# LeSN-Lab/diff-ViT

Measured on AMD Instinct MI355X. Metric: images/sec DeiT-S int8 224^2 b=256 (quantized forward), higher is better.
Workload: dtype int8; 1 GPU; deit_small PoT-PTQ forward, bit_config=[8]*50, 224x224, batch 256 per GPU; global_batch=256, parallelism=dp1, streams_per_gpu=3, collective=none, ranks_seen=1, distinct_devices=1

## Files before the change

diff-vit_amd/csrc/p2vit_attn.hip:

```cpp
#include "p2vit_attn_lis.h"

#define WA_HD 32
#define WA_KEYS 64
#define WA_DEAD(kb, r) (NT > 0 && (kb) * 16 + (r) >= NT)
#define WA_PAD(kb, r) (!(NT > 0 && (kb) * 16 + 12 + (r) < NT))
template <int NT, bool TAP>
__global__ __launch_bounds__(256, 3) void k_window_attention(std::conditional_t<TAP, WinAttnArgs, WinAttnKArgs> a) {
  constexpr int VSTRIDE = WA_KEYS + 4;
  __shared__ __attribute__((aligned(16))) int8_t sK[4][WA_KEYS * WA_HD];
  __shared__ __attribute__((aligned(16))) unsigned short sVt[4][WA_HD * VSTRIDE];
  __shared__ float sT[4][232];
  __shared__ __attribute__((aligned(16))) unsigned short sP[4][4][16];
  __shared__ unsigned short sMeta[WA_KEYS + 16];
  __shared__ long long lutE[258];
  __shared__ double lutFR[258];
  const int tid = threadIdx.x, lane = tid & 63, wave = tid >> 6, g = lane >> 4, l15 = lane & 15;
  const int ws = a.wa.ws, N = ws * ws, nW = a.wa.n_windows;
  const int hgroups = (a.H + 3) >> 2;
  const int blk = blockIdx.x;
  const int hg = blk % hgroups, w = (blk / hgroups) % nW, b = blk / (hgroups * nW);
  const int head = hg * 4 + wave;
  const int C = a.H * WA_HD;
  const long long ldq = a.wa.qkv_stride ? a.wa.qkv_stride : 3 * C, ldo = a.wa.out_stride ? a.wa.out_stride : C;
  const bool hok = head < a.H;
// ... 220 lines not shown
              const int k = (int)((__float_as_uint(ratio[e]) + 0x00400000u) >> 23) - 127;
              const long long trow = (((long long)b * nW + w) * a.H + head) * N + qi;
              if (a.probs_k) a.probs_k[trow * N + kb * 16 + 4 * g + r] = (int8_t)(k > 16 ? 16 : k);
              if (a.probs_kp) a.probs_kp[trow * a.pitch + kb * 16 + 4 * g + r] = (int8_t)(k > 16 ? 16 : k);
            }
          }
          pk[e2] = lis_prob_pair(ratio[0], ratio[1]);
        }
        pb[p] = (v4i){(int)pk[0], (int)pk[1], (int)pk[2], (int)pk[3]};
      }
    }
    v4f o[2] = {(v4f){0.f, 0.f, 0.f, 0.f}, (v4f){0.f, 0.f, 0.f, 0.f}};
#pragma unroll
    for (int p = 0; p < 2; ++p) {
      const v8bf fb = __builtin_bit_cast(v8bf, pb[p]);
#pragma unroll
      for (int dt = 0; dt < 2; ++dt) {
        const unsigned short* vp = &sVt[wave][(dt * 16 + l15) * VSTRIDE + p * 32 + 4 * g];
        const uint2 lo = *reinterpret_cast<const uint2*>(vp);
        const uint2 hi = *reinterpret_cast<const uint2*>(vp + 16);
        v4i va = {(int)lo.x, (int)lo.y, (int)hi.x, (int)hi.y};
        o[dt] = __builtin_amdgcn_mfma_f32_16x16x32_bf16(__builtin_bit_cast(v8bf, va), fb, o[dt], 0, 0, 0);
      }
    }
    if (qi < N) {
      int8_t* dst = a.out + ((long long)b * a.T + rowq) * ldo + head * WA_HD + 4 * g;
#pragma unroll
      for (int dt = 0; dt < 2; ++dt)
        *reinterpret_cast<unsigned*>(dst + dt * 16) = pack4_rne_sat(o[dt][0] * av_mul, o[dt][1] * av_mul, o[dt][2] * av_mul, o[dt][3] * av_mul);
    }
  }
}


int g_attn_waves = 8;
int p2v_launch_window_attention_wide(const WinAttnArgs& a, hipStream_t st);
template <int NT, bool TAP>
static void launch_window_t(const WinAttnArgs& a, dim3 grid, hipStream_t st) {
  hipLaunchKernelGGL((k_window_attention<NT, TAP>), grid, dim3(256), 0, st, a);
}
int p2v_launch_window_attention(const WinAttnArgs& a, hipStream_t st) {
  if (a.wa.ws > 8) return p2v_launch_window_attention_wide(a, st);
  const int hgroups = (a.H + 3) / 4;
  const dim3 grid((unsigned)(a.B * a.wa.n_windows * hgroups));
  static void (*const table[2][2])(const WinAttnArgs&, dim3, hipStream_t) = {{launch_window_t<49, true>, launch_window_t<49, false>},
                                                                             {launch_window_t<0, true>, launch_window_t<0, false>}};
  table[a.wa.ws == 7 ? 0 : 1][a.tapped() ? 0 : 1](a, grid, st);
  CHECK_LAUNCH();
  return 0;
}

int p2v_launch_attention_wide(const AttnArgs& a, int head_dim, int nkb, hipStream_t st);

int g_attn_stream = 0;
int g_attn_packed = 1;
int p2v_attention_kernel_of(int head_dim, int tokens, int tapped) {
  const int resident = p2v_resident_tokens_of(head_dim);
  if (!resident || tokens <= 0 || tokens > P2V_MAX_TOKENS_STREAMED) return -1;
  if (g_attn_stream) return P2V_KERNEL_STREAMING;
  if (tokens <= resident) return P2V_KERNEL_RESIDENT;
  if (g_attn_packed && head_dim == 64 && !tapped && tokens <= P2V_MAX_TOKENS_PACKED) return P2V_KERNEL_PACKED;
  return P2V_KERNEL_STREAMING;
}

int p2v_launch_attention(const AttnArgs& a, int head_dim, hipStream_t st) {
  const int nkb = (a.N + 31) / 32;
  {
    int ex;
    const float m2 = a.at.s_qkv_sq * a.at.inv_s_attn;
    if (!(m2 > 0.f) || frexpf(m2, &ex) != 0.5f) return -2;
  }
  switch (p2v_attention_kernel_of(head_dim, a.N, a.tapped())) {
    case P2V_KERNEL_RESIDENT: break;
    case P2V_KERNEL_PACKED: return p2v_launch_attention_packed(a, st);
    case P2V_KERNEL_STREAMING: return p2v_launch_attention_stream(a, head_dim, st);
    default: return -1;
  }
  if (head_dim == 64) return launch_attn_hd<64, 19, true>(a, nkb, st);
  if (head_dim == 32) return launch_attn_hd<32, 19, false>(a, nkb, st);
  return p2v_launch_attention_wide(a, head_dim, nkb, st);
}
```

diff-vit_amd/csrc/p2vit_attn_lis.h:

```cpp
#pragma once
#include "p2vit_device.h"
#include "p2vit_launch.h"

extern int g_attn_waves;


#define P2V_PROB_SCALE 0x1p111f
__device__ __forceinline__ unsigned lis_prob_pair(float r0, float r1) {
  const unsigned hi2 = __builtin_amdgcn_perm(__float_as_uint(r1), __float_as_uint(r0), 0x07060302u);
  const unsigned eb = __builtin_bit_cast(unsigned, __builtin_bit_cast(v2u16, hi2) + (v2u16){0x40, 0x40}) & 0x7F807F80u;
  unsigned out;
  asm("v_pk_sub_u16 %0, %1, %2 clamp" : "=v"(out) : "s"(0x47804780u), "v"(eb));
  return out;
}

__device__ __forceinline__ void lis_table_entry(const p2v_attn& at, int t, long long* lutE, double* lutFR) {
  if (t >= 256) {
    lutE[256] = 0;
    lutFR[256] = 1.0;
    return;
  }
  int xi = -t;
  const int lim = 32 * at.x0_int;
  xi = xi < lim ? lim : xi;
  const int q = xi / at.x0_int;
  const int r = xi - at.x0_int * q;
  const long long z = (long long)r * (r + at.b_int) + at.c_int;
  long long e = z << (32 - q);
  e = e < 0 ? 0 : e;
  lutE[t] = e;
  lutFR[t] = 1.0 / (double)(float)e;
}

#ifdef P2V_DIAG
extern unsigned long long* g_gemm_stamps;
#define AT_STAMP(slot)                                                                                             \
  do {                                                                                                             \
    if (a.stamps && threadIdx.x == 0 && (slot) < 16) a.stamps[(long long)blockIdx.x * 16 + (slot)] = __builtin_readcyclecounter(); \
  } while (0)
#else
#define AT_STAMP(slot) do { } while (0)
#endif
template <int HD, int NKP, bool TAP, bool ISH>
__global__ __launch_bounds__(512, HD > 64 ? 2 : (NKP <= 7 ? 4 : (NKP <= 10 ? 3 : 2))) void k_lis_attention(std::conditional_t<TAP, AttnArgs, AttnKArgs> a) {
  static_assert(HD % 16 == 0 && HD >= 16 && HD <= 128, "head_dim");
  constexpr int KROWS = NKP * 32;
  constexpr int NKB = NKP * 2;
  constexpr int VSTRIDE = KROWS + 4;
  constexpr int CH = HD / 16;
  constexpr int NQ = (CH + 3) / 4;
  constexpr int NDT = HD / 16;
  extern __shared__ __attribute__((aligned(16))) unsigned char smem[];
  int8_t* sK = reinterpret_cast<int8_t*>(smem);
  unsigned short* sVt = reinterpret_cast<unsigned short*>(smem + KROWS * HD);
  unsigned char* lutE = smem + KROWS * HD + HD * VSTRIDE * 2;
  unsigned char* lutFR = lutE + 258 * 8;
  typedef __attribute__((address_space(3))) const long long* lds_i64p;
  typedef __attribute__((address_space(3))) const double* lds_f64p;
  const int ebase = (int)(unsigned)(uintptr_t)(__attribute__((address_space(3))) unsigned char*)lutE;

  const int tid = threadIdx.x, lane = tid & 63, wave = tid >> 6, g = lane >> 4, l15 = lane & 15;
  const int b = blockIdx.x / a.H, head = blockIdx.x % a.H;
  const int N = a.N, D = a.H * HD, ld = 3 * D;
  const int8_t* base = a.qkv + (long long)b * N * ld + head * HD;
  AT_STAMP(0);

  if (tid < 256) {
    int xi = -tid;
    const int lim = 32 * a.at.x0_int;
    xi = xi < lim ? lim : xi;
    const int q = xi / a.at.x0_int;
    const int r = xi - a.at.x0_int * q;
    const long long z = (long long)r * (r + a.at.b_int) + a.at.c_int;
    long long e = z << (32 - q);
    e = e < 0 ? 0 : e;
    const float ef = (float)e;
    reinterpret_cast<long long*>(lutE)[tid] = e;
    reinterpret_cast<double*>(lutFR)[tid] = 1.0 / (double)ef;
    if (tid == 0) {
      reinterpret_cast<long long*>(lutE)[256] = 0;
      reinterpret_cast<double*>(lutFR)[256] = 1.0;
    }
  }
  AT_STAMP(1);
  for (int i0 = tid; i0 < KROWS * CH; i0 += 2 * (int)blockDim.x) {
    uint4 kv[2], vv[2];
#pragma unroll
    for (int u = 0; u < 2; ++u) {
      const int i = i0 + u * (int)blockDim.x;
      const int row = i / CH, c = i % CH;
      kv[u] = make_uint4(0, 0, 0, 0);
      vv[u] = make_uint4(0, 0, 0, 0);
      if (i < KROWS * CH && row < N) {
        kv[u] = *reinterpret_cast<const uint4*>(base + (long long)row * ld + D + c * 16);
        vv[u] = *reinterpret_cast<const uint4*>(base + (long long)row * ld + 2 * D + c * 16);
      }
    }
#pragma unroll
    for (int u = 0; u < 2; ++u) {
      const int i = i0 + u * (int)blockDim.x;
      if (i >= KROWS * CH) break;
      const int row = i / CH, c = i % CH;
      const int sw = (HD == 64) ? (c ^ (((row >> 3) & 1) << 1)) : c;
      *reinterpret_cast<uint4*>(sK + row * HD + sw * 16) = kv[u];
      const unsigned w4[4] = {vv[u].x, vv[u].y, vv[u].z, vv[u].w};
#pragma unroll
      for (int j = 0; j < 16; ++j) {
        const float f = (float)sx8(w4[j >> 2], j & 3);
        sVt[(c * 16 + j) * VSTRIDE + row] = (unsigned short)(__float_as_uint(f) >> 16);
      }
    }
  }

  const float nmm = -(a.at.qk_scale * (a.at.s_qkv_sq * a.at.inv_s_attn));
  const float avm = a.at.av_mul * P2V_PROB_SCALE;
  const int nqb = ((a.nq > 0 && a.nq < N ? a.nq : N) + 15) >> 4;
  const int nwaves = (int)(blockDim.x >> 6);
  AT_STAMP(2);
  v4i fq_next[NQ];
#pragma unroll
  for (int j = 0; j < NQ; ++j) {
    fq_next[j] = (v4i){0, 0, 0, 0};
    if (4 * j + g < CH && wave < nqb) {
      const int qr0 = wave * 16 + l15;
      fq_next[j] = *reinterpret_cast<const v4i*>(base + (long long)(qr0 < N ? qr0 : N - 1) * ld + (4 * j + g) * 16);
    }
  }
  __syncthreads();
  AT_STAMP(3);
  [[maybe_unused]] int stamp_base = 4;
  for (int qb = wave; qb < nqb; qb += nwaves) {
    const int qrow = qb * 16 + l15;
    v4i fq[NQ];
#pragma unroll
    for (int j = 0; j < NQ; ++j) {
      fq[j] = fq_next[j];
      if (4 * j + g < CH && qb + nwaves < nqb) {
        const int qn = (qb + nwaves) * 16 + l15;
        fq_next[j] = *reinterpret_cast<const v4i*>(base + (long long)(qn < N ? qn : N - 1) * ld + (4 * j + g) * 16);
      }
    }
    v4i s[NKB];
#pragma unroll
    for (int kb = 0; kb < NKB; ++kb) {
      const int row = kb * 16 + l15;
#pragma unroll
      for (int j = 0; j < NQ; ++j) {
        const bool live = 4 * j + g < CH;
        const int c = live ? 4 * j + g : 0;
        const int sw = (HD == 64) ? (c ^ (((row >> 3) & 1) << 1)) : c;
        v4i fk = *reinterpret_cast<const v4i*>(sK + row * HD + sw * 16);
        if (!live) fk = (v4i){0, 0, 0, 0};
        if (j == 0) s[kb] = __builtin_amdgcn_mfma_i32_16x16x64_i8(fk, fq[0], (v4i){0, 0, 0, 0}, 0, 0, 0);
        else s[kb] = __builtin_amdgcn_mfma_i32_16x16x64_i8(fk, fq[j], s[kb], 0, 0, 0);
      }
    }
    const bool tail_empty = (NKB - 1) * 16 >= N;
#ifdef P2V_DIAG
    asm volatile("s_nop 0" :: "v"(s[NKB - 1][0]));
#endif
    AT_STAMP(stamp_base);
    long long S = 0;
    [[maybe_unused]] int rowmax = 0;
    if (ISH) {
      const int p = a.pshift, hm1 = (1 << (p - 1)) - 1;
      int mx = -100000;
#pragma unroll
      for (int kb = 0; kb < NKB; ++kb) {
        if (kb == NKB - 1 && tail_empty) continue;
#pragma unroll
        for (int r = 0; r < 4; ++r) {
          const int sv = s[kb][r];
          int code = (int)((unsigned)sv + (unsigned)hm1 + (((unsigned)sv >> p) & 1u)) >> p;
          code = code < -128 ? -128 : (code > 127 ? 127 : code);
          if (kb >= NKB - 2) code = (kb * 16 + 4 * g + r) < N ? code : -100000;
          s[kb][r] = code;
          mx = code > mx ? code : mx;
        }
      }
      {
        int o = __shfl_xor(mx, 16);
        mx = o > mx ? o : mx;
        o = __shfl_xor(mx, 32);
        mx = o > mx ? o : mx;
      }
      if (TAP) rowmax = mx;
      const int mx8 = (mx << 3) + ebase;
#pragma unroll
      for (int kb = 0; kb < NKB; ++kb) {
        if (kb == NKB - 1 && tail_empty) continue;
#pragma unroll
        for (int r = 0; r < 4; ++r) {
          int d8;
          asm("v_mad_i32_i24 %0, %1, -8, %2" : "=v"(d8) : "v"(s[kb][r]), "v"(mx8));
          if (kb >= NKB - 2) d8 = d8 > ebase + 2048 ? ebase + 2048 : d8;
          s[kb][r] = d8;
          S += *(lds_i64p)(uintptr_t)(unsigned)d8;
        }
        __builtin_amdgcn_sched_barrier(0);
      }
    } else {
    int mn = 1000;
#pragma unroll
    for (int kb = 0; kb < NKB; ++kb) {
      if (kb == NKB - 1 && tail_empty) continue;
#pragma unroll
      for (int r = 0; r < 4; ++r) {
        int nc = (int)__builtin_amdgcn_fmed3f(rintf((float)s[kb][r] * nmm), -127.f, 128.f);
        if (kb >= NKB - 2) nc = (kb * 16 + 4 * g + r) < N ? nc : 1000;
        s[kb][r] = nc;
        mn = nc < mn ? nc : mn;
      }
    }
    {
      int o = __shfl_xor(mn, 16);
      mn = o < mn ? o : mn;
      o = __shfl_xor(mn, 32);
      mn = o < mn ? o : mn;
    }
    if (TAP) rowmax = -mn;
    const int neg8mn = -8 * mn + ebase;
#pragma unroll
    for (int kb = 0; kb < NKB; ++kb) {
      if (kb == NKB - 1 && tail_empty) continue;
#pragma unroll
      for (int r = 0; r < 4; ++r) {
        int d8 = (s[kb][r] << 3) + neg8mn;
        if (kb >= NKB - 2) d8 = d8 > ebase + 2048 ? ebase + 2048 : d8;
        s[kb][r] = d8;
        S += *(lds_i64p)(uintptr_t)(unsigned)d8;
      }
      __builtin_amdgcn_sched_barrier(0);
    }
    }
    S += __shfl_xor(S, 16);
    S += __shfl_xor(S, 32);
    const float Sf = (float)S;
    const double Sd = (double)Sf;
    AT_STAMP(stamp_base + 1);

// ... 99 lines not shown
```

diff-vit_amd/csrc/p2vit_capi.cpp:

```cpp
#include <hip/hip_runtime.h>
#include <math.h>
#include <stdarg.h>
#include <stdio.h>
#include <stdlib.h>
#include <string.h>

#include <initializer_list>
#include <memory>
#include <vector>

#include "p2vit_kernels.h"

static thread_local char g_err[512] = "";

static int fail(int code, const char* fmt, ...) {
  va_list ap;
  va_start(ap, fmt);
  vsnprintf(g_err, sizeof g_err, fmt, ap);
  va_end(ap);
  return code;
}
struct KeepLastError {
  char keep[sizeof g_err];
  KeepLastError() { memcpy(keep, g_err, sizeof keep); }
// ... 7 lines not shown
}
static inline int round_up(int v, int m) { return (v + m - 1) / m * m; }
static bool is_pot(float v) {
  int ex;
  return v > 0.f && frexpf(v, &ex) == 0.5f;
}

static int check_lis_consts(const char* who, int x0_int, int b_int, int c_int) {
  if (x0_int >= 0) return fail(P2V_E_ARG, "%s: x0_int must be negative", who);
  if (c_int <= 0 || c_int >= (1 << 24) || b_int < 0 || b_int >= (1 << 23) || x0_int < -(1 << 12))
    return fail(P2V_E_UNSUPPORTED, "%s: log-int-softmax constants out of range (x0 %d, b %d, c %d): softmax input scale below 2^-11?", who, x0_int,
                b_int, c_int);
  return P2V_OK;
}
static int check_requant_scale(const char* who, float inv_s_out) {
  if (!(is_pot(inv_s_out) && inv_s_out >= 0x1p-40f && inv_s_out <= 0x1p40f))
    return fail(P2V_E_UNSUPPORTED, "%s: REQUANT 1/scale %g must be a power of two (it is folded into the column scales)", who, inv_s_out);
  return P2V_OK;
}
static int check_gelu_tab(const char* who, const p2v_gelu_tab& t) {
  if (t.table && (t.cells <= 0 || t.cells > 4096)) return fail(P2V_E_ARG, "%s: GELU table with %d cells", who, t.cells);
  return P2V_OK;
}
static int check_attn(const char* who, const p2v_attn& at) {
  const int rc = check_lis_consts(who, at.x0_int, at.b_int, at.c_int);
  if (rc != P2V_OK) return rc;
  if (!is_pot(at.s_qkv_sq * at.inv_s_attn)) return fail(P2V_E_UNSUPPORTED, "%s: s_qkv_sq * inv_s_attn must be a power of two", who);
  if (!(at.qk_scale > 0.f) || !(at.av_mul > 0.f)) return fail(P2V_E_ARG, "%s: qk_scale and av_mul must be positive", who);
  if (!is_pot(at.av_mul) || at.av_mul > 0x1p15f || at.av_mul < 0x1p-40f)
    return fail(P2V_E_UNSUPPORTED, "%s: av_mul %g must be a power of two in [2^-40, 2^15]", who, at.av_mul);
  return P2V_OK;
}

struct p2v_plan {
  p2v_model_desc d;
  int tokens, patches, k_patch, k_patch_pad, n_layers;
  std::vector<p2v_linear> lin[2];
  std::vector<char> lin_set[2];
  float inv_s_input;
  p2v_epilogue embed_epi;
  const int8_t* cls_codes;
  const int8_t* embed_cls_codes = nullptr;
  bool embed_set;
  std::vector<p2v_block> blocks;
  std::vector<char> block_set;
  p2v_ln final_ln;
  float head_inv_s, head_s;
  bool head_set;
  std::vector<float*> ln_pre_buf;
  float* final_pre_buf = nullptr;
  std::vector<char> block_folded;
  std::vector<const float*> resid_tab;
  std::vector<float*> resid_buf;
  int device = -1;
  ~p2v_plan() {
    int prev = -1;
    const bool sw = device >= 0 && hipGetDevice(&prev) == hipSuccess && prev != device && hipSetDevice(device) == hipSuccess;
    for (float* b : ln_pre_buf)
      if (b) (void)hipFree(b);
    for (float* b : resid_buf)
      if (b) (void)hipFree(b);
    if (final_pre_buf) (void)hipFree(final_pre_buf);
    if (sw) (void)hipSetDevice(prev);
  }
};

static void build_resid_tables(p2v_plan* plan, int block);
static int bit_index(int bits) { return bits == 4 ? 0 : (bits == 8 ? 1 : -1); }
template <class Block>
static auto& block_ln(Block& b, int i) { return i < 2 ? b.ln1[i] : b.ln2[(i - 2) >> 1][(i - 2) & 1]; }
static bool ln_constants_present(const p2v_ln& l, bool with_mask = true) {
  return (l.mask || !with_mask) && l.gamma && l.beta && l.inv_out && l.post_mul;
}

extern "C" {

extern int g_ln_generic;
extern int g_ln_rows;
extern int g_attn_waves;
extern int g_ln_gemm;
extern int g_ln_gemm_ver;
extern int g_gemm_tile;
extern int g_resid_pre;
extern int g_attn_stream;
extern int g_attn_packed;
extern int g_ln_pre;
extern int g_gemm_rows;
int g_cls_rows = 1;

enum { ANY_ENV = 1, ANY_API = 2 };
static const struct Switch {
  const char *name, *env;
  int* var;
  int lo, hi, step, any;
  bool takes(int v, int how) const { return (any & how) || (v >= lo && v <= hi && (v - lo) % step == 0); }
  void set(int v) const { *var = (hi == 1 && lo == 0) ? v != 0 : v; }
} kSwitches[] = {
    {"attn_waves", "P2V_ATTN_WAVES", &g_attn_waves, 4, 8, 1, 0},
    {"ln_gemm", "P2V_LN_GEMM", &g_ln_gemm, 0, 1, 1, ANY_ENV | ANY_API},
    {"ln_gemm_version", "P2V_LN_GEMM_V", &g_ln_gemm_ver, 1, 3, 1, 0},
    {"gemm_tile", "P2V_GEMM_TILE", &g_gemm_tile, 0, 256, 128, 0},
    {"attn_stream", "P2V_ATTN_STREAM", &g_attn_stream, 0, 1, 1, ANY_ENV | ANY_API},
    {"attn_packed", "P2V_ATTN_PACKED", &g_attn_packed, 0, 1, 1, 0},
    {"ln_pre", "P2V_LN_PRE", &g_ln_pre, 0, 1, 1, ANY_ENV | ANY_API},
    {"resid_pre", "P2V_RESID_PRE", &g_resid_pre, 0, 1, 1, ANY_ENV | ANY_API},
    {"gemm_rows", "P2V_GEMM_ROWS", &g_gemm_rows, 0, 2, 1, 0},
    {"cls_rows", "P2V_CLS_ROWS", &g_cls_rows, 0, 1, 1, ANY_ENV},
    {"ln_rows", "P2V_LN_ROWS", &g_ln_rows, 1, 64, 1, 0},
    {"ln_generic", "P2V_LN_GENERIC", &g_ln_generic, 0, 1, 1, ANY_API},
};

static void read_env_once() {
  static bool done = false;
  if (done) return;
  done = true;
  for (const Switch& s : kSwitches) {
    const char* e = getenv(s.env);
    if (e && s.takes(atoi(e), ANY_ENV)) s.set(atoi(e));
  }
}
int p2v_abi_version(void) { read_env_once(); return P2V_ABI_VERSION; }

int p2v_resident_tokens(int head_dim) { return p2v_resident_tokens_of(head_dim); }
int p2v_max_tokens(int head_dim) { return p2v_resident_tokens_of(head_dim) ? P2V_MAX_TOKENS_STREAMED : 0; }
int p2v_packed_tokens(int head_dim) { return head_dim == 64 ? P2V_MAX_TOKENS_PACKED : 0; }
int p2v_attention_kernel(int head_dim, int tokens, int tapped) {
  read_env_once();
  return p2v_attention_kernel_of(head_dim, tokens, tapped);
}

int p2v_set_tuning(const char* name, int value) {
  if (!name) return fail(P2V_E_ARG, "p2v_set_tuning: null name");
  read_env_once();
  for (const Switch& s : kSwitches)
    if (!strcmp(name, s.name) && s.takes(value, ANY_API)) {
      s.set(value);
      return P2V_OK;
    }
  return fail(P2V_E_ARG, "p2v_set_tuning: unknown switch or value out of range: %s = %d", name, value);
}
const char* p2v_last_error(void) { return g_err; }

int p2v_plan_create(const p2v_model_desc* desc, p2v_plan** out) {
  if (!desc || !out) return fail(P2V_E_ARG, "p2v_plan_create: null argument");
  read_env_once();
  if (desc->abi_version != P2V_ABI_VERSION) return fail(P2V_E_ARG, "ABI version %d != %d", desc->abi_version, P2V_ABI_VERSION);
  const p2v_model_desc& d = *desc;
  if (d.img_size <= 0 || d.patch_size <= 0 || d.img_size % d.patch_size) return fail(P2V_E_SHAPE, "img_size %% patch_size != 0");
  if (d.patch_size % 4) return fail(P2V_E_UNSUPPORTED, "patch_size must be a multiple of 4");
  if (d.embed_dim % d.num_heads) return fail(P2V_E_SHAPE, "embed_dim %% num_heads != 0");
  const int hd = d.embed_dim / d.num_heads;
  if (hd != 32 && hd != 48 && hd != 64 && hd != 80 && hd != 96 && hd != 128)
    return fail(P2V_E_UNSUPPORTED, "head_dim %d (32, 48, 64, 80, 96 and 128 are instantiated)", hd);
  if (d.embed_dim % 16 || d.mlp_hidden % 16) return fail(P2V_E_UNSUPPORTED, "embed_dim and mlp_hidden must be multiples of 16");
  {
    const int tokens = (d.img_size / d.patch_size) * (d.img_size / d.patch_size) + 1;
    if (tokens > P2V_MAX_TOKENS_STREAMED)
      return fail(P2V_E_UNSUPPORTED, "%d tokens per image: the attention kernels cover up to %d", tokens, P2V_MAX_TOKENS_STREAMED);
  }
  if (d.embed_dim > 2048) return fail(P2V_E_UNSUPPORTED, "embed_dim %d: the LayerNorm kernel covers up to 2048 channels", d.embed_dim);
  p2v_plan* p = new p2v_plan();
  p->d = d;
  p->patches = (d.img_size / d.patch_size) * (d.img_size / d.patch_size);
  p->tokens = p->patches + 1;
  p->k_patch = d.in_chans * d.patch_size * d.patch_size;
  p->k_patch_pad = round_up(p->k_patch, GBK_PAD);
  p->n_layers = 4 * d.depth + 2;
  for (int b = 0; b < 2; ++b) {
    p->lin[b].assign(p->n_layers, p2v_linear{nullptr, nullptr, nullptr, nullptr, 0});
    p->lin_set[b].assign(p->n_layers, 0);
  }
  p->blocks.resize(d.depth);
  p->block_set.assign(d.depth, 0);
  p->ln_pre_buf.assign(d.depth, nullptr);
  p->block_folded.assign(d.depth, 0);
  p->resid_tab.assign((size_t)d.depth * 4, nullptr);
  p->resid_buf.assign(d.depth, nullptr);
  p->embed_set = p->head_set = false;
  p->cls_codes = nullptr;
  *out = p;
  return P2V_OK;
}

void p2v_plan_destroy(p2v_plan* plan) { delete plan; }

int p2v_plan_set_linear(p2v_plan* plan, int layer, int bits, const p2v_linear* lin) {
  if (!plan || !lin) return fail(P2V_E_ARG, "p2v_plan_set_linear: null argument");
  const int bi = bit_index(bits);
  if (bi < 0) return fail(P2V_E_BITS, "bits %d not in {4, 8}", bits);
  if (layer < 0 || layer >= plan->n_layers) return fail(P2V_E_ARG, "layer %d out of range [0,%d)", layer, plan->n_layers);
  if (!lin->w_codes || !lin->colscale || !lin->bias) return fail(P2V_E_ARG, "p2v_plan_set_linear: null device pointer");
  if (lin->packed4 && bits != 4) return fail(P2V_E_BITS, "packed4 weights for a %d-bit layer", bits);
  plan->lin[bi][layer] = *lin;
  plan->lin_set[bi][layer] = 1;
  if (layer >= 1 && layer < plan->n_layers - 1 && ((layer - 1) & 1)) {
    const int block = (layer - 1) / 4;
    if (plan->block_set[block]) build_resid_tables(plan, block);
  }
  return P2V_OK;
}

int p2v_plan_set_embed(p2v_plan* plan, float inv_s_input, const p2v_epilogue* e, const int8_t* cls_row_codes) {
  if (!plan || !e || !cls_row_codes) return fail(P2V_E_ARG, "p2v_plan_set_embed: null argument");
  plan->inv_s_input = inv_s_input;
  plan->embed_epi = *e;
  plan->embed_epi.patches = plan->patches;
  plan->cls_codes = cls_row_codes;
  plan->embed_set = true;
  return P2V_OK;
}

int p2v_plan_set_embed_tap_cls(p2v_plan* plan, const int8_t* cls_embed_codes) {
  if (!plan || !cls_embed_codes) return fail(P2V_E_ARG, "p2v_plan_set_embed_tap_cls: null argument");
  plan->embed_cls_codes = cls_embed_codes;
  return P2V_OK;
}

struct OwnerDevice {
  int prev = -1, own = -1;
  explicit OwnerDevice(const void* ptr) {
    hipPointerAttribute_t pa;
    if (hipGetDevice(&prev) != hipSuccess || hipPointerGetAttributes(&pa, ptr) != hipSuccess) {
      (void)hipGetLastError();
      return;
    }
    if (pa.type != hipMemoryTypeDevice && pa.type != hipMemoryTypeManaged) return;
    own = pa.device;
    if (own != prev && hipSetDevice(own) != hipSuccess) own = -1;
  }
  ~OwnerDevice() { if (own >= 0 && own != prev) (void)hipSetDevice(prev); }
// ... 62 lines not shown
  float gmin = 3.0e38f, gmax = 0.f, bmax = 0.f;
  for (int c = 0; c < C; ++c) {
    unsigned ib;
    memcpy(&ib, &io[c], 4);
    const int p2 = (int)((ib & 0x807FFFFFu) == 0u) & (int)((ib >> 23) - 32u <= 190u);
    go[c] = g[c] * io[c];
    bo[c] = b[c] * io[c];
    const float ga = fabsf(go[c]), ba = fabsf(bo[c]);
    const int gok = (int)(g[c] == 0.f) | ((int)(ga >= 1.0e-30f) & (int)(ga <= 1.0e30f));
    const int bok = (int)(b[c] == 0.f) | ((int)(ba >= 1.0e-30f) & (int)(ba <= 1.0e30f));
    pot &= p2 & gok & bok;
    pm1 &= (int)(pm[c] == 1.f);
    gmin = fminf(gmin, ga);
    gmax = fmaxf(gmax, ga);
    bmax = fmaxf(bmax, ba);
  }
  e = hipMemcpy(dev, host.data(), host.size() * sizeof(float), hipMemcpyHostToDevice);
  if (e == hipSuccess) *out = p2v_ln_pre{dev, dev + Cp, gmin, gmax, bmax, pot, pm1};
  return e;
}
static const p2v_ln_pre kNoPre = {nullptr, nullptr, 0.f, 0.f, 0.f, 0, 0};

static bool fold_ln_constants(p2v_plan* plan, int block) {
  const int C = plan->d.embed_dim, Cp = round_up(C, 256);
  p2v_block& blk = plan->blocks[block];
  for (int i = 0; i < 6; ++i) block_ln(blk, i).pre = kNoPre;
  OwnerDevice own(blk.ln1[0].gamma);
  if (!own.ok()) {
    fail(P2V_OK, "p2v_plan_set_block: LayerNorm constants of block %d not folded at plan time (cannot locate the device of gamma)", block);
    return false;
  }
  if (plan->device >= 0 && plan->device != own.own) {
    fail(P2V_OK, "p2v_plan_set_block: block %d lives on device %d, earlier blocks on device %d: not folded at plan time", block, own.own, plan->device);
    return false;
  }
  hipError_t e = hipDeviceSynchronize();
  float* dev = plan->ln_pre_buf[block];
  if (e == hipSuccess && !dev) e = hipMalloc(&dev, (size_t)12 * Cp * sizeof(float));
  p2v_ln_pre pre[6];
  if (e == hipSuccess) {
    plan->ln_pre_buf[block] = dev;
    plan->device = own.own;
    for (int i = 0; i < 6 && e == hipSuccess; ++i) e = fold_one_ln(block_ln(blk, i), C, dev + (size_t)(2 * i) * Cp, &pre[i]);
  }
  if (e != hipSuccess) {
    (void)hipGetLastError();
    fail(P2V_OK, "p2v_plan_set_block: LayerNorm constants of block %d not folded at plan time (%s)", block, hipGetErrorString(e));
    return false;
  }
  for (int i = 0; i < 6; ++i) block_ln(blk, i).pre = pre[i];
  return true;
}

int p2v_plan_set_block(p2v_plan* plan, int block, const p2v_block* blk) {
  if (!plan || !blk) return fail(P2V_E_ARG, "p2v_plan_set_block: null argument");
  if (block < 0 || block >= plan->d.depth) return fail(P2V_E_ARG, "block %d out of range", block);
  int rc = check_attn("p2v_plan_set_block: attn", blk->attn);
  if (rc == P2V_OK) rc = check_gelu_tab("p2v_plan_set_block: gelu_fc1", blk->gelu_fc1);
  for (int b = 0; b < 2 && rc == P2V_OK; ++b) rc = check_requant_scale("p2v_plan_set_block: inv_s_qkv", blk->inv_s_qkv[b]);
  if (rc == P2V_OK && !(is_pot(blk->inv_s_fc1) && blk->inv_s_fc1 >= 0x1p-40f && blk->inv_s_fc1 <= 0x1p40f))
    rc = fail(P2V_E_UNSUPPORTED, "p2v_plan_set_block: 1/scale of mlp.qact1 %g must be a power of two", blk->inv_s_fc1);
  if (rc == P2V_OK && (!blk->proj_epi.s_mid || !blk->proj_epi.s_res || !blk->proj_epi.s_next || !blk->fc2_epi.s_mid || !blk->fc2_epi.s_res ||
                       !blk->fc2_epi.s_next))
    rc = fail(P2V_E_ARG, "p2v_plan_set_block: RESID epilogues need s_mid/s_res/s_next");
  for (int i = 0; i < 6 && rc == P2V_OK; ++i)
    if (!ln_constants_present(block_ln(*blk, i))) rc = fail(P2V_E_ARG, "p2v_plan_set_block: LayerNorm constants missing");
  if (rc != P2V_OK) return rc;
  plan->blocks[block] = *blk;
  plan->block_set[block] = 1;
  g_err[0] = 0;
  plan->block_folded[block] = fold_ln_constants(plan, block) ? 1 : 0;
  build_resid_tables(plan, block);
  return P2V_OK;
}

int p2v_plan_block_prefolded(const p2v_plan* plan, int block) {
  if (!plan || block < 0 || block >= plan->d.depth) return fail(P2V_E_ARG, "p2v_plan_block_prefolded: bad argument");
  return plan->block_folded[block] ? 1 : 0;
}

int p2v_plan_resid_prefolded(const p2v_plan* plan, int block) {
  if (!plan || block < 0 || block >= plan->d.depth) return fail(P2V_E_ARG, "p2v_plan_resid_prefolded: bad argument");
  int m = 0;
  for (int j = 0; j < 4; ++j) m |= plan->resid_tab[(size_t)block * 4 + j] ? 1 << j : 0;
  return m;
}

int p2v_plan_set_head(p2v_plan* plan, const p2v_ln* final_ln, float inv_s_out, float s_out) {
  if (!plan || !final_ln) return fail(P2V_E_ARG, "p2v_plan_set_head: null argument");
  if (!ln_constants_present(*final_ln))
    return fail(P2V_E_ARG, "p2v_plan_set_head: LayerNorm constants missing");
  if (!(inv_s_out > 0.f) || !(s_out > 0.f)) return fail(P2V_E_ARG, "p2v_plan_set_head: act_out scale must be positive");
  plan->final_ln = *final_ln;
  plan->final_ln.pre = kNoPre;
  {
    OwnerDevice own(final_ln->gamma);
    const int C = plan->d.embed_dim;
    if (own.ok() && (plan->device < 0 || plan->device == own.own) && hipDeviceSynchronize() == hipSuccess) {
      if (!plan->final_pre_buf && hipMalloc(&plan->final_pre_buf, (size_t)2 * round_up(C, 256) * sizeof(float)) != hipSuccess) plan->final_pre_buf = nullptr;
      p2v_ln_pre pre;
      if (plan->final_pre_buf && fold_one_ln(*final_ln, C, plan->final_pre_buf, &pre) == hipSuccess) {
        plan->final_ln.pre = pre;
        plan->device = own.own;
      }
    }
    (void)hipGetLastError();
  }
  plan->head_inv_s = inv_s_out;
  plan->head_s = s_out;
  plan->head_set = true;
  return P2V_OK;
}

struct WsLayout {
  size_t patches, x, ln, qkv, att, hid, cls, total;
};
static WsLayout ws_layout(const p2v_plan* p, int batch) {
  auto al = [](size_t v) { return (v + 255) / 256 * 256; };
  const size_t M = (size_t)batch * p->tokens, D = p->d.embed_dim;
  WsLayout w;
  size_t off = 0;
  w.patches = off; off += al((size_t)batch * p->patches * p->k_patch_pad);
  w.x = off;       off += al(M * D);
  w.ln = off;      off += al(M * D);
  w.qkv = off;     off += al(M * 3 * D);
// ... 128 lines not shown
      if (prof->used + 1 >= (int)prof->ev.size()) return fail(P2V_E_LAUNCH, "profile: event pool exhausted");
      hipEventRecord(prof->ev[prof->used++], st);
      prof->kind.push_back(kind);
    }
    const int rc = launch();
    if (rc == P2V_OK) launched += (kind == P2V_K_LN_GEMM_QKV || kind == P2V_K_LN_GEMM_FC1) ? 2 : 1;
    return rc;
  }
  int lin_tap(int layer, const int8_t* A, int lda, int rows, int K, int N, const p2v_linear& lin) {
    if (done || !o.lin_tap || !o.lin_tap[layer]) return P2V_OK;
    return run_gemm(P2V_EPI_F32, A, lda, rows, K, N, lin, p2v_epilogue{}, o.lin_tap[layer], N, nullptr, st);
  }
  int ddv_i8(const void* buf, int rows, int cols, const float* scale) { return (done || !o.ddv) ? P2V_OK : ddv_reduce(o.ddv, buf, rows, cols, P2V_COS_I8, scale, st); }
  int ddv_f32(const void* buf, int rows, int cols) { return (done || !o.ddv) ? P2V_OK : ddv_reduce(o.ddv, buf, rows, cols, P2V_COS_F32, nullptr, st); }
  int ddv_i8_deq(const void* buf, int rows, int cols, const float* scale) { return (done || !o.ddv) ? P2V_OK : ddv_reduce(o.ddv, buf, rows, cols, P2V_COS_I8_DEQ, scale, st); }
  int ddv_tap(int rows, int cols) { return (o.ddv && o.ddv->tap) ? ddv_f32(o.ddv->tap, rows, cols) : P2V_OK; }
  float* full() const { return (!done && o.ddv) ? o.ddv->scratch : nullptr; }
  int layernorm(const LnArgs& a) { return step(P2V_K_LAYERNORM, [&] { return launch_rc(p2v_launch_layernorm(a, st), "int_layernorm"); }); }
  int gemm(int kind, bool few, int epi, const int8_t* A, int lda, int rows, int K, int N, const p2v_linear& lin, const p2v_epilogue& ep, void* out, int ldo,
           int8_t* out_codes = nullptr) {
    return step(kind, [&] { return run_gemm(epi, A, lda, rows, K, N, lin, ep, out, ldo, out_codes, st, few); });
  }
  int ln_linear(int k_fused, int k_gemm, int epi, long long stride, int rows, const p2v_ln& norm, const p2v_linear& lin, const p2v_epilogue& e, int N,
                int8_t* out, bool few) {
    LnArgs ln{X, stride, rows, D, norm, LN, D};
    ln.pre = norm.pre;
    if (float* vals = full()) {
      ln.tap_out = vals;
      int rc = layernorm(ln);
      if (rc || (rc = ddv_f32(vals, T, D))) return rc;
      return gemm(k_gemm, few, epi, LN, D, rows, Dk, N, lin, e, out, N);
    }
    if (!few && lin.w_frag && p2v_ln_gemm_supported(epi, D, N, e.gelu.table ? e.gelu.cells : 0)) {
      if (o.stop_after < 0) ln.out = nullptr;
      return step(k_fused, [&] { return run_ln_gemm(epi, ln, lin, e, N, out, st); });
    }
    const int rc = layernorm(ln);
    return rc ? rc : gemm(k_gemm, few, epi, LN, D, rows, Dk, N, lin, e, out, N);
  }

  int block(int i, const int8_t* bc, const RowSet& rs) {
    const p2v_block& b = p->blocks[i];
    const int bq = bit_index(bc[0]), bp = bit_index(bc[1]), b1 = bit_index(bc[2]), b2 = bit_index(bc[3]);
    const p2v_linear &qkv = p->lin[bq][1 + 4 * i], &proj = p->lin[bp][2 + 4 * i], &fc1 = p->lin[b1][3 + 4 * i], &fc2 = p->lin[b2][4 + 4 * i];
    const int ldx = (int)rs.stride;
    int rc;
    p2v_epilogue eq{};
    eq.inv_s_out = b.inv_s_qkv[bq];
    eq.tap_out = o.qkv_tap ? o.qkv_tap[i] : (o.lin_tap ? o.lin_tap[1 + 4 * i] : nullptr);
    if ((rc = ln_linear(P2V_K_LN_GEMM_QKV, P2V_K_GEMM_QKV, P2V_EPI_REQUANT, D, M, b.ln1[bq], qkv, eq, 3 * D, QKV, false))) return rc;
    if ((rc = ddv_tap(T, 3 * D)) || (rc = ddv_i8(QKV, T, 3 * D, nullptr))) return rc;
    AttnArgs at{{QKV, batch, T, p->d.num_heads, b.attn, ATT, nullptr}};
    at.nq = rs.nq;
    int8_t* planes = (!done && o.ddv) ? o.ddv->attn : nullptr;
    const int pitch = round_up(T, 16), HT = p->d.num_heads * T;
    if (planes) {
      at.score_codes = planes;
      at.probs_kp = planes + (size_t)batch * HT * pitch;
      at.pitch = pitch;
    }
    if ((rc = step(P2V_K_ATTENTION, [&] { return launch_rc(p2v_launch_attention(at, hd, st), "lis_attention"); }))) return rc;
    if (planes && !done &&
        ((rc = ddv_reduce(o.ddv, at.score_codes, HT, T, P2V_COS_I8, nullptr, st, 0, pitch)) ||
         (rc = ddv_reduce(o.ddv, at.probs_kp, HT, T, P2V_COS_LOG2K, nullptr, st, 0, pitch))))
      return rc;
    if ((rc = ddv_i8(ATT, T, D, nullptr))) return rc;
    p2v_epilogue ep = b.proj_epi;
    ep.residual = X;
    ep.resid_tab = p->resid_tab[(size_t)i * 4 + bp];
    if ((rc = gemm(P2V_K_GEMM_PROJ, rs.few, P2V_EPI_RESID, ATT, ldx, rs.rows, Dk, D, proj, ep, X, ldx, full() ? LN : nullptr))) return rc;
    if ((rc = lin_tap(2 + 4 * i, ATT, ldx, rs.rows, Dk, D, proj)) || (rc = ddv_tap(T, D))) return rc;
    if (full() && (rc = ddv_i8_deq(LN, T, D, b.proj_epi.s_mid))) return rc;
    if ((rc = ddv_i8(X, T, D, b.proj_epi.s_next))) return rc;
    p2v_epilogue e1{};
    e1.inv_s_out = b.inv_s_fc1;
    e1.gelu = b.gelu_fc1;
    e1.tap_out = o.fc1_tap ? o.fc1_tap[i] : (o.lin_tap ? o.lin_tap[3 + 4 * i] : nullptr);
    if ((rc = ln_linear(P2V_K_LN_GEMM_FC1, P2V_K_GEMM_FC1, P2V_EPI_GELU, rs.stride, rs.rows, b.ln2[bq][b1], fc1, e1, Hd, HID, rs.few))) return rc;
    if ((rc = ddv_tap(T, Hd)) || (rc = ddv_i8(HID, T, Hd, nullptr))) return rc;
    p2v_epilogue e2 = b.fc2_epi;
    e2.residual = X;
    e2.resid_tab = p->resid_tab[(size_t)i * 4 + 2 + b2];
    if ((rc = gemm(P2V_K_GEMM_FC2, rs.few, P2V_EPI_RESID, HID, Hd, rs.rows, Hk, D, fc2, e2, X, ldx, full() ? LN : nullptr))) return rc;
    if ((rc = lin_tap(4 + 4 * i, HID, Hd, rs.rows, Hk, D, fc2)) || (rc = ddv_tap(T, D))) return rc;
    if (full() && (rc = ddv_i8_deq(LN, T, D, b.fc2_epi.s_mid))) return rc;
    return ddv_i8(X, T, D, b.fc2_epi.s_next);
  }
};

static int forward_impl(p2v_plan* p, int batch, const int8_t* bit_config, int n_cfg, float* logits, void* workspace, size_t workspace_bytes,
                        void* stream, const FwdOpts& o) {
  if (!p || !(o.images || o.u8) || !bit_config || !logits || !workspace) return fail(P2V_E_ARG, "p2v_forward: null argument");
  if (batch <= 0) return fail(P2V_E_SHAPE, "batch must be positive");
  if (n_cfg != p->n_layers) return fail(P2V_E_BITS, "bit_config has %d entries, model needs %d", n_cfg, p->n_layers);
  for (int i = 0; i < n_cfg; ++i) {
    const int bi = bit_index(bit_config[i]);
    if (bi < 0) return fail(P2V_E_BITS, "%d is not in list", (int)bit_config[i]);
    if (!p->lin_set[bi][i]) return fail(P2V_E_STATE, "layer %d has no %d-bit weights", i, (int)bit_config[i]);
  }
  if (!p->embed_set || !p->head_set) return fail(P2V_E_STATE, "plan incomplete (embed/head)");
  for (int i = 0; i < p->d.depth; ++i)
    if (!p->block_set[i]) return fail(P2V_E_STATE, "plan incomplete (block %d)", i);
  const WsLayout w = ws_layout(p, batch);
  if (workspace_bytes < w.total) return fail(P2V_E_WORKSPACE, "workspace %zu < %zu bytes", workspace_bytes, w.total);
  if (o.lin_tap && o.lin_tap[0] && !(p->inv_s_input > 0.f))
    return fail(P2V_E_UNSUPPORTED, "p2v_forward_linear_taps: no patch-embed tap for input_quant = False (the fp32-image convolution); pass NULL for taps[0]");
// ... 873 lines not shown
```

diff-vit_amd/csrc/p2vit_kernels.h:

```cpp
#pragma once
#include <hip/hip_runtime.h>
#include <stdint.h>

#include "../../include/p2vit.h"

#define GBK_PAD 64
#define P2V_EPI_F32 7

struct GemmArgs {
  const int8_t* A;
  int lda, M;
  const int8_t* W;
  int K, N;
  int w4;
  const float* colscale;
  const float* bias;
  p2v_epilogue ep;
  void* out;
  int ldo;
  int8_t* out_codes;
  int8_t* out_codes2;
  int tiles_n;
#ifdef P2V_DIAG
  unsigned long long* stamps;
#endif
};

typedef p2v_ln_pre LnPre;

struct LnArgs {
  const int8_t* x;
  long long row_stride;
  long long rows;
  int C;
  p2v_ln ln;
  int8_t* out;
  long long out_stride;
  int rows_per_half;
  int force_generic;
  LnPre pre;
  float* tap_out;
};

struct AttnKArgs {
  const int8_t* qkv;
  int B, N, H;
  p2v_attn at;
  int8_t* out;
  int8_t* probs_k;
  int pshift;
  int nq;
#ifdef P2V_DIAG
  unsigned long long* stamps;
#endif
};
struct AttnArgs : AttnKArgs {
  int8_t* score_codes;
  int8_t* probs_kp;
  int pitch;
  bool tapped() const { return probs_k || score_codes || probs_kp; }
};

struct WinAttnKArgs {
  const int8_t* qkv;
  int B, T, H;
  p2v_winattn wa;
  int8_t* out;
  int8_t* probs_k;
};
struct WinAttnArgs : WinAttnKArgs {
  int8_t* attn1_codes;
  int8_t* qact2_codes;
  int8_t* probs_kp;
  int pitch;
  bool tapped() const { return probs_k || attn1_codes || qact2_codes || probs_kp; }
};
int p2v_launch_patch_merge_gather(const int8_t* x, int B, int H, int W, int C, int8_t* out, hipStream_t st);
int p2v_launch_avgpool_quant(const int8_t* x, int B, int T, int C, float s_in, float inv_s_out, int8_t* out, hipStream_t st);
int p2v_launch_window_attention(const WinAttnArgs& a, hipStream_t st);

int p2v_launch_patchify(const float* img, int B, int C, int H, int W, int P, float inv_s, int8_t* out, int k_pad, hipStream_t st);
int p2v_launch_fill_cls(int8_t* x, int B, int T, int D, const int8_t* cls, hipStream_t st);
int p2v_launch_embed_fp32(const float* img, int B, int C, int H, int W, int P, const GemmArgs& g, hipStream_t st);
int p2v_launch_u8_patchify(const uint8_t* img, int B, int C, int H, int W, int P, int nhwc, const int8_t* lut, int8_t* out, int k_pad,
                           hipStream_t st);
int p2v_launch_embed_u8(const uint8_t* img, int nhwc, const float* lut, int B, int C, int H, int W, int P, const GemmArgs& g, hipStream_t st);
int p2v_launch_gemm(int epi, const GemmArgs& g, hipStream_t st);
int p2v_launch_gemm_rows(int epi, const GemmArgs& g, hipStream_t st);
int p2v_launch_resid_prefold(const p2v_linear& lin, const p2v_epilogue& ep, int N, float* tab, unsigned* flags, hipStream_t st);
#define P2V_LN_MAX_C 4096
int p2v_launch_layernorm(const LnArgs& a, hipStream_t st);
int p2v_launch_layernorm_xwide(const LnArgs& a, hipStream_t st);
bool p2v_ln_gemm_supported(int epi, int C, int N, int table_cells);
int p2v_launch_ln_gemm(int epi, const LnArgs& a, const GemmArgs& g, hipStream_t st);
int p2v_launch_attention(const AttnArgs& a, int head_dim, hipStream_t st);
int p2v_launch_attention_stream(const AttnArgs& a, int head_dim, hipStream_t st);
int p2v_launch_attention_packed(const AttnArgs& a, hipStream_t st);
int p2v_attention_kernel_of(int head_dim, int tokens, int tapped);
inline int p2v_resident_tokens_of(int head_dim) {
  if (head_dim == 32 || head_dim == 48 || head_dim == 64 || head_dim == 80) return P2V_MAX_TOKENS;
  return head_dim == 96 ? 17 * 32 : (head_dim == 128 ? 12 * 32 : 0);
}
int p2v_launch_stream_probe(int kernels, int usec, int workgroups, int lds_bytes, hipStream_t st);
int p2v_launch_fake_quant(const float* x, long long n, const float* scale, int n_scale, long long inner, int lo, int hi,
                          float* out, int8_t* codes, hipStream_t st);
int p2v_launch_gelu_quant(const float* y, long long n, float inv_s, int8_t* codes, unsigned long long* flags, int force_slow,
                          hipStream_t st);
int p2v_launch_gelu_sweep(unsigned first_bits, unsigned count, float* max_err, hipStream_t st);
// ... 64 lines not shown
```

Before: 108,600 images/sec.

## Precompute attention exp LUT per block and use float-magic softmax requantization

Builds the per-block exponent/reciprocal lookup tables once at plan setup in a global buffer, and has the attention kernel copy them into LDS instead of recomputing them with integer division and double reciprocal in every workgroup. The copy is split so one load overlaps the K/V staging. Score requantization is also rewritten to use an fma with a magic constant plus med3 clamp on float bits, replacing the integer rounding shift and clamp sequence. This adds a global read per workgroup and a setup kernel with device syncs at plan time.

New measurement: 109,600 images/sec, median of 6. No clear change (+0.9%).

```diff
diff --git a/diff-vit_amd/csrc/p2vit_attn.hip b/diff-vit_amd/csrc/p2vit_attn.hip
--- a/diff-vit_amd/csrc/p2vit_attn.hip
+++ b/diff-vit_amd/csrc/p2vit_attn.hip
@@ -296,6 +296,24 @@
 
 int p2v_launch_attention_wide(const AttnArgs& a, int head_dim, int nkb, hipStream_t st);
 
+__global__ __launch_bounds__(320) void k_lis_tables(p2v_attn at, unsigned char* img) {
+  const int t = threadIdx.x;
+  long long* lutE = reinterpret_cast<long long*>(img);
+  double* lutFR = reinterpret_cast<double*>(img + P2V_ATTN_LUT_BYTES / 2);
+  if (t < 257) {
+    lis_table_entry(at, t, lutE, lutFR);
+  } else if (t == 257) {
+    lutE[257] = 0;
+    lutFR[257] = 0.0;
+  }
+}
+int p2v_launch_lis_tables(const p2v_attn& at, void* img, hipStream_t st) {
+  hipLaunchKernelGGL(k_lis_tables, dim3(1), dim3(320), 0, st, at, static_cast<unsigned char*>(img));
+  CHECK_LAUNCH();
+  return 0;
+}
+
+int g_attn_lut = 1;
 int g_attn_stream = 0;
 int g_attn_packed = 1;
 int p2v_attention_kernel_of(int head_dim, int tokens, int tapped) {
diff --git a/diff-vit_amd/csrc/p2vit_attn_lis.h b/diff-vit_amd/csrc/p2vit_attn_lis.h
--- a/diff-vit_amd/csrc/p2vit_attn_lis.h
+++ b/diff-vit_amd/csrc/p2vit_attn_lis.h
@@ -65,22 +65,12 @@
   const int8_t* base = a.qkv + (long long)b * N * ld + head * HD;
   AT_STAMP(0);
 
-  if (tid < 256) {
-    int xi = -tid;
-    const int lim = 32 * a.at.x0_int;
-    xi = xi < lim ? lim : xi;
-    const int q = xi / a.at.x0_int;
-    const int r = xi - a.at.x0_int * q;
-    const long long z = (long long)r * (r + a.at.b_int) + a.at.c_int;
-    long long e = z << (32 - q);
-    e = e < 0 ? 0 : e;
-    const float ef = (float)e;
-    reinterpret_cast<long long*>(lutE)[tid] = e;
-    reinterpret_cast<double*>(lutFR)[tid] = 1.0 / (double)ef;
-    if (tid == 0) {
-      reinterpret_cast<long long*>(lutE)[256] = 0;
-      reinterpret_cast<double*>(lutFR)[256] = 1.0;
-    }
+  const uint4* lutg = reinterpret_cast<const uint4*>(a.lut);
+  uint4 lutv = make_uint4(0, 0, 0, 0);
+  if (lutg) {
+    if (tid < 258) lutv = lutg[tid];
+  } else if (tid < 257) {
+    lis_table_entry(a.at, tid, reinterpret_cast<long long*>(lutE), reinterpret_cast<double*>(lutFR));
   }
   AT_STAMP(1);
   for (int i0 = tid; i0 < KROWS * CH; i0 += 2 * (int)blockDim.x) {
@@ -112,6 +102,11 @@
     }
   }
 
+  if (lutg) {
+    if (tid < 258) reinterpret_cast<uint4*>(lutE)[tid] = lutv;
+    for (int t = tid + (int)blockDim.x; t < 258; t += (int)blockDim.x) reinterpret_cast<uint4*>(lutE)[t] = lutg[t];
+  }
+
   const float nmm = -(a.at.qk_scale * (a.at.s_qkv_sq * a.at.inv_s_attn));
   const float avm = a.at.av_mul * P2V_PROB_SCALE;
   const int nqb = ((a.nq > 0 && a.nq < N ? a.nq : N) + 15) >> 4;
@@ -163,20 +158,21 @@
     long long S = 0;
     [[maybe_unused]] int rowmax = 0;
     if (ISH) {
-      const int p = a.pshift, hm1 = (1 << (p - 1)) - 1;
-      int mx = -100000;
+      constexpr int MBITS = 0x4B400000, PADBITS = MBITS - 100000;
+      const float sc = __uint_as_float((unsigned)(127 - a.pshift) << 23), Mf = __int_as_float(MBITS);
+      int mx = PADBITS;
 #pragma unroll
       for (int kb = 0; kb < NKB; ++kb) {
         if (kb == NKB - 1 && tail_empty) continue;
 #pragma unroll
         for (int r = 0; r < 4; ++r) {
-          const int sv = s[kb][r];
-          int code = (int)((unsigned)sv + (unsigned)hm1 + (((unsigned)sv >> p) & 1u)) >> p;
-          code = code < -128 ? -128 : (code > 127 ? 127 : code);
-          if (kb >= NKB - 2) code = (kb * 16 + 4 * g + r) < N ? code : -100000;
-          s[kb][r] = code;
-          mx = code > mx ? code : mx;
+          const float t = __builtin_amdgcn_fmed3f(__builtin_fmaf((float)s[kb][r], sc, Mf), Mf - 128.f, Mf + 127.f);
+          int bits = __float_as_int(t);
+          if (kb >= NKB - 2) bits = (kb * 16 + 4 * g + r) < N ? bits : PADBITS;
+          s[kb][r] = bits;
+          mx = bits > mx ? bits : mx;
         }
+        if constexpr (NKP > 10) __builtin_amdgcn_sched_barrier(0);
       }
       {
         int o = __shfl_xor(mx, 16);
@@ -184,8 +180,8 @@
         o = __shfl_xor(mx, 32);
         mx = o > mx ? o : mx;
       }
-      if (TAP) rowmax = mx;
-      const int mx8 = (mx << 3) + ebase;
+      if (TAP) rowmax = mx - MBITS;
+      const int mx8 = ((mx - 0x4B000000) << 3) + ebase;
 #pragma unroll
       for (int kb = 0; kb < NKB; ++kb) {
         if (kb == NKB - 1 && tail_empty) continue;
diff --git a/diff-vit_amd/csrc/p2vit_capi.cpp b/diff-vit_amd/csrc/p2vit_capi.cpp
--- a/diff-vit_amd/csrc/p2vit_capi.cpp
+++ b/diff-vit_amd/csrc/p2vit_capi.cpp
@@ -83,6 +83,8 @@
   std::vector<char> block_folded;
   std::vector<const float*> resid_tab;
   std::vector<float*> resid_buf;
+  unsigned char* attn_lut_buf = nullptr;
+  std::vector<const void*> attn_lut;
   int device = -1;
   ~p2v_plan() {
     int prev = -1;
@@ -92,6 +94,7 @@
     for (float* b : resid_buf)
       if (b) (void)hipFree(b);
     if (final_pre_buf) (void)hipFree(final_pre_buf);
+    if (attn_lut_buf) (void)hipFree(attn_lut_buf);
     if (sw) (void)hipSetDevice(prev);
   }
 };
@@ -115,6 +118,7 @@
 extern int g_resid_pre;
 extern int g_attn_stream;
 extern int g_attn_packed;
+extern int g_attn_lut;
 extern int g_ln_pre;
 extern int g_gemm_rows;
 int g_cls_rows = 1;
@@ -133,6 +137,7 @@
     {"gemm_tile", "P2V_GEMM_TILE", &g_gemm_tile, 0, 256, 128, 0},
     {"attn_stream", "P2V_ATTN_STREAM", &g_attn_stream, 0, 1, 1, ANY_ENV | ANY_API},
     {"attn_packed", "P2V_ATTN_PACKED", &g_attn_packed, 0, 1, 1, 0},
+    {"attn_lut", "P2V_ATTN_LUT", &g_attn_lut, 0, 1, 1, 0},
     {"ln_pre", "P2V_LN_PRE", &g_ln_pre, 0, 1, 1, ANY_ENV | ANY_API},
     {"resid_pre", "P2V_RESID_PRE", &g_resid_pre, 0, 1, 1, ANY_ENV | ANY_API},
     {"gemm_rows", "P2V_GEMM_ROWS", &g_gemm_rows, 0, 2, 1, 0},
@@ -207,6 +212,7 @@
   p->block_folded.assign(d.depth, 0);
   p->resid_tab.assign((size_t)d.depth * 4, nullptr);
   p->resid_buf.assign(d.depth, nullptr);
+  p->attn_lut.assign(d.depth, nullptr);
   p->embed_set = p->head_set = false;
   p->cls_codes = nullptr;
   *out = p;
@@ -375,6 +381,26 @@
   return true;
 }
 
+static void build_attn_lut(p2v_plan* plan, int block) {
+  KeepLastError keep;
+  plan->attn_lut[block] = nullptr;
+  const p2v_block& blk = plan->blocks[block];
+  OwnerDevice dev(blk.ln1[0].gamma);
+  if (!dev.ok() || (plan->device >= 0 && plan->device != dev.own)) return;
+  if (!plan->attn_lut_buf && hipMalloc(&plan->attn_lut_buf, (size_t)plan->d.depth * P2V_ATTN_LUT_BYTES) != hipSuccess) {
+    (void)hipGetLastError();
+    plan->attn_lut_buf = nullptr;
+    return;
+  }
+  plan->device = dev.own;
+  unsigned char* img = plan->attn_lut_buf + (size_t)block * P2V_ATTN_LUT_BYTES;
+  if (hipDeviceSynchronize() != hipSuccess || p2v_launch_lis_tables(blk.attn, img, nullptr) != 0 || hipDeviceSynchronize() != hipSuccess) {
+    (void)hipGetLastError();
+    return;
+  }
+  plan->attn_lut[block] = img;
+}
+
 int p2v_plan_set_block(p2v_plan* plan, int block, const p2v_block* blk) {
   if (!plan || !blk) return fail(P2V_E_ARG, "p2v_plan_set_block: null argument");
   if (block < 0 || block >= plan->d.depth) return fail(P2V_E_ARG, "block %d out of range", block);
@@ -394,6 +420,7 @@
   g_err[0] = 0;
   plan->block_folded[block] = fold_ln_constants(plan, block) ? 1 : 0;
   build_resid_tables(plan, block);
+  build_attn_lut(plan, block);
   return P2V_OK;
 }
 
@@ -628,6 +655,7 @@
     if ((rc = ddv_tap(T, 3 * D)) || (rc = ddv_i8(QKV, T, 3 * D, nullptr))) return rc;
     AttnArgs at{{QKV, batch, T, p->d.num_heads, b.attn, ATT, nullptr}};
     at.nq = rs.nq;
+    at.lut = g_attn_lut ? p->attn_lut[i] : nullptr;
     int8_t* planes = (!done && o.ddv) ? o.ddv->attn : nullptr;
     const int pitch = round_up(T, 16), HT = p->d.num_heads * T;
     if (planes) {
diff --git a/diff-vit_amd/csrc/p2vit_kernels.h b/diff-vit_amd/csrc/p2vit_kernels.h
--- a/diff-vit_amd/csrc/p2vit_kernels.h
+++ b/diff-vit_amd/csrc/p2vit_kernels.h
@@ -53,7 +53,10 @@
 #ifdef P2V_DIAG
   unsigned long long* stamps;
 #endif
+  const void* lut = nullptr;
 };
+#define P2V_ATTN_LUT_BYTES (2 * 258 * 8)
+int p2v_launch_lis_tables(const p2v_attn& at, void* img, hipStream_t st);
 struct AttnArgs : AttnKArgs {
   int8_t* score_codes;
   int8_t* probs_kp;
```
